# imulki/serenade

Measured on AMD Instinct MI355X. Metric: mel frames/sec converted (UNet ODE + vocoder), 80x1024, higher is better.
Workload: dtype f32

## Files before the change

### include/serenade_hip.h

```cpp
#ifndef SERENADE_HIP_H
#define SERENADE_HIP_H

#include <stdint.h>

#ifdef __cplusplus
extern "C" {
#endif

#define SRN_ABI_VERSION 4
#define SRN_MAX_TAPS 16

enum { SRN_ACT_NONE = 0, SRN_ACT_LEAKY = 1, SRN_ACT_SILU = 2, SRN_ACT_MISH = 3 };
enum { SRN_RES_NONE = 0, SRN_RES_ADD = 1, SRN_RES_AXPY = 2 };
enum {
  SRN_POST_NONE = 0,
  SRN_POST_DIV = 1,
  SRN_POST_TANH = 2,
  SRN_POST_RELU = 3,
  SRN_POST_LEAKY = 4,
  SRN_POST_GELU = 5
};
enum {
  SRN_PREC_FP32 = 0,
  SRN_PREC_BF16X3 = 1,
// ... 53 lines not shown
  void* ws; int64_t ws_bytes;
  const void* w_hi; const void* w_lo;
  float* gn_partials;
  float* out_tr; int64_t out_tr_bs; int32_t ld_out_tr; int32_t out_tr_col0;
} SrnConvParams;

int srn_abi_version(void);
const char* srn_last_error(void);

int srn_conv_gemm(const SrnConvParams* p, void* stream);
int64_t srn_conv_gemm_workspace_bytes(const SrnConvParams* p);
int srn_conv_gemm_route(const SrnConvParams* p, int32_t out[3]);
#define SRN_FORM_FIELDS 9
int srn_conv_gemm_forms(int32_t* rows, int capacity);

int srn_gn_mish_apply(const float* x, const float* gn_partials, const float* gamma, const float* beta,
                      const float* time_bias, int64_t time_bias_bs, const int32_t* lens, float* y, int B, int T,
                      int C, int groups, float eps, int valid_stats, void* stream);

int srn_resblock_tail(const float* c2, const float* gn_partials, const float* gamma, const float* beta,
                      const int32_t* lens, const float* r, const float* scale, const float* shift, int64_t ld_ss,
                      float* y, int B, int T, int C, int groups, float gn_eps, float ln_eps, int valid_stats,
                      void* stream);

int srn_resblock_tail_ln(const float* c2, const float* gn_partials, const float* gamma, const float* beta,
                         const int32_t* lens, const float* r, const float* scale, const float* shift, int64_t ld_ss,
                         float* y, int B, int T, int C, int groups, float gn_eps, float ln_eps, int valid_stats,
                         const float* ln2_gamma, const float* ln2_beta, float* y2, float ln2_eps, void* stream);

int srn_layernorm(const float* x, const float* gamma, const float* beta, float* y, int64_t rows, int C, float eps,
                  void* stream);

int srn_softmax_rows(float* s, const int32_t* lens, int Z, int n_head, int L, int ld, void* stream);

int srn_sinusoidal_emb(const float* t, float* out, int n, int dim, int ld, float scale, void* stream);

int srn_copy_channels(const float* src, int64_t src_bs, int ld_src, int sc0, float* dst, int64_t dst_bs, int ld_dst,
                      int dc0, int B, int T, int C, void* stream);

int srn_scatter_rows(const float* src, int64_t src_bs, int ld_src, float* dst, int64_t dst_bs, int ld_dst, int dc0,
                     const int32_t* row_off, const int32_t* n_rows, int B, int T, int C, void* stream);

int srn_transpose_ct(const float* src, float* dst, int B, int R, int Cc, int64_t src_bs, int ld_src, int64_t dst_bs,
                     int ld_dst, void* stream);
#define SRN_TR_LIST_MAX 40
typedef struct SrnTransposeList {
  int32_t n;
  int32_t pad_;
  const float* src[SRN_TR_LIST_MAX];
  float* dst[SRN_TR_LIST_MAX];
  int64_t src_bs[SRN_TR_LIST_MAX], dst_bs[SRN_TR_LIST_MAX];
  int32_t B[SRN_TR_LIST_MAX], R[SRN_TR_LIST_MAX], Cc[SRN_TR_LIST_MAX];
  int32_t ld_src[SRN_TR_LIST_MAX], ld_dst[SRN_TR_LIST_MAX];
  int32_t first_block[SRN_TR_LIST_MAX + 1];
} SrnTransposeList;
int srn_transpose_multi(const SrnTransposeList* list, void* stream);

int srn_renorm(const float* x, const float* trg_scale, const float* trg_mean, const float* voc_mean,
               const float* voc_scale, float* y, int64_t rows, int C, void* stream);

int srn_out_conv_tanh(const float* x, const float* w, const float* bias, float* y, int B, int T, int C, int k,
                      float slope, void* stream);
int srn_out_conv_tanh_ragged(const float* x, const float* w, const float* bias, float* y, const int32_t* lens, int B,
                             int T, int C, int k, float slope, void* stream);

typedef struct SrnResUnitParams {
// ... 256 lines not shown
```

### serenade_amd/_lib.py

```python
import collections
import ctypes
import os
from ctypes import POINTER, c_char_p, c_double, c_float, c_int, c_int32, c_int64, c_void_p

_HERE = os.path.dirname(os.path.abspath(__file__))
LIB_PATH = os.environ.get("SERENADE_AMD_LIB") or os.path.join(_HERE, "libserenade_hip.so")

SRN_MAX_TAPS = 16
ACT_NONE, ACT_LEAKY, ACT_SILU, ACT_MISH = 0, 1, 2, 3
RES_NONE, RES_ADD, RES_AXPY = 0, 1, 2
POST_NONE, POST_DIV, POST_TANH, POST_RELU, POST_LEAKY, POST_GELU = 0, 1, 2, 3, 4, 5
PREC_FP32, PREC_BF16X3, PREC_BF16X6 = 0, 1, 2
ROUTE_AUTO, ROUTE_TILED, ROUTE_HALO, ROUTE_GENERIC, ROUTE_STRIP, ROUTE_FAST_FP32 = 0, 1, 2, 3, 4, 5
FAMILY_GENERIC, FAMILY_F32, FAMILY_FAST, FAMILY_HALO, FAMILY_STRIP = 0, 1, 2, 3, 4
RESUNIT_ROUTE_SHARED = 1
TN_ROUTE_GENERAL = 1
RESUNIT_FORM_F32, RESUNIT_FORM_SHARED_F32, RESUNIT_FORM_BF16X3 = 0, 1, 2


class SrnConvParams(ctypes.Structure):
    _fields_ = [
        ("n_batch", c_int32), ("n_head", c_int32), ("T_in", c_int32), ("T_out", c_int32),
        ("C_in", c_int32), ("C_in0", c_int32), ("C_w", c_int32), ("N", c_int32), ("N_out", c_int32),
        ("n_taps", c_int32), ("tap_off", c_int32 * SRN_MAX_TAPS), ("in_stride", c_int32),
# ... 66 lines not shown
        ("route", c_int32),
    ]


class SrnExcitationParams(ctypes.Structure):
    _fields_ = [
        ("n_batch", c_int32), ("max_frames", c_int32), ("fs", c_int32), ("hop", c_int32),
        ("f0", c_void_p), ("df_f0", c_void_p), ("f_bs", c_int64), ("n_frames", c_void_p), ("phase_ws", c_void_p),
        ("noise", c_void_p), ("sine", c_void_p), ("sine_amp", c_float), ("noise_amp", c_float), ("n_df", c_int32),
        ("dfs", c_void_p * 4), ("df_upsample", c_int32 * 4), ("dense_factors", c_double * 4),
    ]


_P = c_void_p
_SIGS = {
    "srn_abi_version": (c_int, []),
    "srn_last_error": (c_char_p, []),
    "srn_conv_gemm": (c_int, [POINTER(SrnConvParams), _P]),
    "srn_conv_gemm_workspace_bytes": (c_int64, [POINTER(SrnConvParams)]),
    "srn_conv_gemm_route": (c_int, [POINTER(SrnConvParams), POINTER(c_int32)]),
    "srn_conv_gemm_forms": (c_int, [POINTER(c_int32), c_int]),
    "srn_hifigan_resunit": (c_int, [POINTER(SrnResUnitParams), _P]),
    "srn_hifigan_resunit_route": (c_int, [POINTER(SrnResUnitParams), POINTER(c_int32)]),
    "srn_hifigan_resunit_ragged": (c_int, [POINTER(SrnResUnitParams), _P, _P]),
    "srn_hifigan_resunit_ragged_route": (c_int, [POINTER(SrnResUnitParams), _P, POINTER(c_int32)]),
    "srn_gn_mish_apply": (c_int, [_P, _P, _P, _P, _P, c_int64, _P, _P, c_int, c_int, c_int, c_int, c_float, c_int, _P]),
    "srn_resblock_tail": (c_int, [_P, _P, _P, _P, _P, _P, _P, _P, c_int64, _P, c_int, c_int, c_int, c_int,
                                  c_float, c_float, c_int, _P]),
    "srn_resblock_tail_ln": (c_int, [_P, _P, _P, _P, _P, _P, _P, _P, c_int64, _P, c_int, c_int, c_int, c_int,
                                     c_float, c_float, c_int, _P, _P, _P, c_float, _P]),
    "srn_scatter_rows": (c_int, [_P, c_int64, c_int, _P, c_int64, c_int, c_int, _P, _P, c_int, c_int, c_int, _P]),
    "srn_layernorm": (c_int, [_P, _P, _P, _P, c_int64, c_int, c_float, _P]),
    "srn_softmax_rows": (c_int, [_P, _P, c_int, c_int, c_int, c_int, _P]),
    "srn_sinusoidal_emb": (c_int, [_P, _P, c_int, c_int, c_int, c_float, _P]),
    "srn_copy_channels": (c_int, [_P, c_int64, c_int, c_int, _P, c_int64, c_int, c_int, c_int, c_int, c_int, _P]),
    "srn_transpose_ct": (c_int, [_P, _P, c_int, c_int, c_int, c_int64, c_int, c_int64, c_int, _P]),
    "srn_transpose_multi": (c_int, [POINTER(SrnTransposeList), _P]),
    "srn_weight_norm_fwd": (c_int, [_P, _P, _P, _P, _P, c_int, c_int, c_int, _P]),
    "srn_weight_norm_bwd": (c_int, [_P, _P, _P, _P, _P, _P, c_int, c_int, c_int, _P]),
    "srn_renorm": (c_int, [_P, _P, _P, _P, _P, _P, c_int64, c_int, _P]),
    "srn_out_conv_tanh": (c_int, [_P, _P, _P, _P, c_int, c_int, c_int, c_int, c_float, _P]),
    "srn_out_conv_tanh_ragged": (c_int, [_P, _P, _P, _P, _P, c_int, c_int, c_int, c_int, c_float, _P]),
    "srn_pd_gather": (c_int, [_P, _P, _P, c_int, c_int, c_int, c_float, c_float, _P]),
    "srn_pd_gather_ragged": (c_int, [_P, _P, _P, _P, c_int, c_int, c_int, c_float, c_float, _P]),
    "srn_pad_signal": (c_int, [_P, _P, c_int, c_int, c_int, c_int, c_int, _P]),
    "srn_logmel": (c_int, [_P, _P, _P, c_int64, c_int, c_int, c_int, c_float, c_int, _P]),
    "srn_loudness": (c_int, [_P, _P, _P, _P, c_int, c_int, c_int, c_int, c_float, c_float, c_float, _P]),
    "srn_pad_ragged_zero": (c_int, [_P, c_int64, _P, _P, c_int, c_int, c_int, c_int, _P]),
    "srn_logmel_ragged": (c_int, [_P, _P, _P, _P, c_int, c_int, c_int, c_int, c_int, c_float, c_int, _P]),
    "srn_loudness_ragged": (c_int, [_P, _P, _P, _P, _P, c_int, c_int, c_int, c_int, c_float, c_float, c_float, _P]),
    "srn_gru_recur_last": (c_int, [_P, _P, _P, _P, c_int, c_int, c_int, _P]),
    "srn_style_token_attention_kv": (c_int, [_P] * 8 + [c_int] * 5 + [_P]),
    "srn_rowln_fwd": (c_int, [_P, _P, c_int64, _P, c_int64, _P, c_int, c_int, c_int, c_float, _P]),
    "srn_rowln_bwd": (c_int, [_P, _P, _P, c_int64, _P, _P, c_int, c_int, c_int, c_float, _P]),
    "srn_rowln_chunks": (c_int, [c_int]),
    "srn_gn_mish_bwd_partial": (c_int, [_P] * 8 + [c_int] * 4 + [_P]),
    "srn_gn_mish_bwd_apply": (c_int, [_P] * 9 + [c_int] * 4 + [_P]),
    "srn_gn_chunks": (c_int, [c_int]),
    "srn_gn_stats": (c_int, [_P, _P, _P, c_int, c_int, c_int, c_int, c_float, _P]),
    "srn_chunk_colsum": (c_int, [_P, _P, _P, _P, c_int, c_int, c_int, c_int, _P]),
    "srn_colsum": (c_int, [_P, _P, _P, c_int, c_int64, c_int, c_int, _P]),
    "srn_colsum_chunks": (c_int, [c_int64]),
    "srn_softmax_bwd": (c_int, [_P, _P, c_int64, c_int, c_int, c_float, _P]),
    "srn_geglu_fwd": (c_int, [_P, _P, c_int64, c_int, _P]),
    "srn_geglu_bwd": (c_int, [_P, _P, _P, c_int64, c_int, _P]),
    "srn_adamw": (c_int, [_P, _P, _P, _P, c_int64, c_float, c_float, c_float, c_float, c_float, c_int, c_float, _P]),
# ... 48 lines not shown
    "srn_note_decode": (c_int, [_P] * 4 + [c_int] * 3 + [c_float] * 2 + [c_int, c_double] + [_P] * 7),
    "srn_note_frames": (c_int, [_P] * 3 + [c_int] * 2 + [_P] + [c_double] * 3 + [_P] * 4 + [c_int] + [_P] * 3),
}

EXPORTS = tuple(_SIGS)

_lib = None


def lib():
    global _lib
    if _lib is None:
        if not os.path.exists(LIB_PATH):
            raise RuntimeError(
                f"{LIB_PATH} not found: build it with `python -m serenade_amd.build` "
                "(hipcc --offload-arch=gfx950). There is no CPU fallback.")
        h = ctypes.CDLL(LIB_PATH)
        for name, (res, args) in _SIGS.items():
            fn = getattr(h, name)
            fn.restype = res
            fn.argtypes = args
        if h.srn_abi_version() != 4:
            raise RuntimeError("libserenade_hip.so ABI version mismatch")
        _lib = h
    return _lib


def check(rc, what=""):
    if rc != 0:
        msg = lib().srn_last_error().decode("utf-8", "replace")
        raise RuntimeError(f"libserenade_hip {what} failed (rc={rc}): {msg}")


ConvForm = collections.namedtuple("ConvForm", "family tile precision nmajor kslices bm bn wn stages")


def conv_forms():
    k = len(ConvForm._fields)
    n = lib().srn_conv_gemm_forms(None, 0)
    rows = (c_int32 * (n * k))()
    assert lib().srn_conv_gemm_forms(rows, n) == n
    return [ConvForm(*rows[i * k:(i + 1) * k]) for i in range(n)]
```

### serenade_amd/csrc/norm_act.hip

```cpp
#include "common.h"
#include "conv_common.h"
#include "row_common.h"

namespace {

__device__ __forceinline__ void group_stats(const float* __restrict__ partials, int b, int T, int C, int groups,
                                            float eps, float* s_mean, float* s_rstd, int n_rows) {
  gn_group_stats(partials, b, T, C, groups, eps, n_rows,
                 [&](int g, float mean, float rstd) { s_mean[g] = mean, s_rstd[g] = rstd; });
  __syncthreads();
}

constexpr int GN_ROWS = 8;
constexpr int SMALL_GRID = 512;
constexpr int GN_PRE = 4;

__global__ __launch_bounds__(256) void gn_mish_apply_kernel(const float* __restrict__ x,
                                                            const float* __restrict__ partials,
                                                            const float* __restrict__ gamma,
                                                            const float* __restrict__ beta,
                                                            const float* __restrict__ time_bias,
                                                            const int32_t* __restrict__ lens, float* __restrict__ y,
                                                            int T, int C, int groups, float eps, int64_t tb_bs,
                                                            int valid_stats, int rows_per_wg) {
  __shared__ float s_mean[64], s_rstd[64];
  const int b = blockIdx.y;
  const int r0 = blockIdx.x * rows_per_wg;
  if (time_bias) time_bias += (int64_t)b * tb_bs;
  const int len = lens ? min(lens[b], T) : T;
  const int c4n = C / 4;
  const int cpg = C / groups;
  const int rows = min(rows_per_wg, T - r0);
  const int total = rows * c4n;
  const int64_t base = ((int64_t)b * T + r0) * C;
  float4 pre[GN_PRE];
#pragma unroll
  for (int k = 0; k < GN_PRE; ++k) {
    const int idx = threadIdx.x + 256 * k;
    pre[k] = make_float4(0.f, 0.f, 0.f, 0.f);
    if (idx < total) {
      const int r = idx / c4n;
      if (r0 + r < len) pre[k] = *reinterpret_cast<const float4*>(x + base + (int64_t)r * C + (idx - r * c4n) * 4);
    }
  }
  group_stats(partials, b, T, C, groups, eps, s_mean, s_rstd, valid_stats ? len : T);
  auto one = [&](const int idx, const float4 v) {
    const int r = idx / c4n;
    const int c = (idx - r * c4n) * 4;
    float4 o = make_float4(0.f, 0.f, 0.f, 0.f);
    if (r0 + r < len) {
      const float4 ga = *reinterpret_cast<const float4*>(gamma + c);
      const float4 be = *reinterpret_cast<const float4*>(beta + c);
      const int g = c / cpg;
      o = gn_mish4(v, s_mean[g], s_rstd[g], ga, be);
      if (time_bias) {
        const float4 tb = *reinterpret_cast<const float4*>(time_bias + c);
        o.x += tb.x;
        o.y += tb.y;
        o.z += tb.z;
        o.w += tb.w;
      }
    }
    *reinterpret_cast<float4*>(y + base + (int64_t)r * C + c) = o;
  };
#pragma unroll
  for (int k = 0; k < GN_PRE; ++k)
    if ((int)threadIdx.x + 256 * k < total) one(threadIdx.x + 256 * k, pre[k]);
  for (int idx = threadIdx.x + 256 * GN_PRE; idx < total; idx += 256) {
    const int r = idx / c4n;
    float4 v = make_float4(0.f, 0.f, 0.f, 0.f);
    if (r0 + r < len) v = *reinterpret_cast<const float4*>(x + base + (int64_t)r * C + (idx - r * c4n) * 4);
    one(idx, v);
  }
}

constexpr int TAIL_ROWS = 8;

__global__ __launch_bounds__(256) void resblock_tail_kernel(
    const float* __restrict__ c2, const float* __restrict__ partials, const float* __restrict__ gamma,
    const float* __restrict__ beta, const int32_t* __restrict__ lens, const float* __restrict__ rres,
    const float* __restrict__ scale, const float* __restrict__ shift, int64_t ld_ss, float* __restrict__ y, int T,
    int C, int groups, float gn_eps, float ln_eps, int valid_stats, const float* __restrict__ ln2_gamma,
    const float* __restrict__ ln2_beta, float* __restrict__ y2, float ln2_eps, int rows_per_wg) {
  __shared__ float s_mean[64], s_rstd[64];
  const int b = blockIdx.y;
  const int r0 = blockIdx.x * rows_per_wg;
  const int len = lens ? min(lens[b], T) : T;
  const int wave = threadIdx.x >> 6, lane = threadIdx.x & 63;
  const int c4n = C / 4;
  const int cpg = C / groups;
  const float inv_c = 1.0f / (float)C;
  const int r_end = min(r0 + rows_per_wg, T);
  float4 xin[MAXV], rin[MAXV];
  auto fetch = [&](const int r) {
    const int64_t row = ((int64_t)b * T + r) * C;
#pragma unroll
    for (int i = 0; i < MAXV; ++i) {
      const int c4 = lane + 64 * i;
      xin[i] = rin[i] = make_float4(0.f, 0.f, 0.f, 0.f);
      if (c4 < c4n) {
        rin[i] = *reinterpret_cast<const float4*>(rres + row + c4 * 4);
        if (r < len) xin[i] = *reinterpret_cast<const float4*>(c2 + row + c4 * 4);
      }
    }
  };
  if (r0 + wave < r_end) fetch(r0 + wave);
  group_stats(partials, b, T, C, groups, gn_eps, s_mean, s_rstd, valid_stats ? len : T);
  for (int r = r0 + wave; r < r_end; r += 4) {
    if (r != r0 + wave) fetch(r);
    const int64_t row = ((int64_t)b * T + r) * C;
    const bool valid = r < len;
    float4 v[MAXV];
#pragma unroll
    for (int i = 0; i < MAXV; ++i) {
      const int c4 = lane + 64 * i;
      v[i] = make_float4(0.f, 0.f, 0.f, 0.f);
      if (c4 < c4n) {
        const int c = c4 * 4;
        const float4 rr = rin[i];
        float4 o = make_float4(0.f, 0.f, 0.f, 0.f);
        if (valid) {
          const float4 ga = *reinterpret_cast<const float4*>(gamma + c);
          const float4 be = *reinterpret_cast<const float4*>(beta + c);
          const int g = c / cpg;
          o = gn_mish4(xin[i], s_mean[g], s_rstd[g], ga, be);
        }
        v[i] = make_float4(o.x + rr.x, o.y + rr.y, o.z + rr.z, o.w + rr.w);
      }
    }
    const float mean = row_sum(v, lane, c4n) * inv_c;
    const float stdv = sqrtf(row_sqdev(v, mean, lane, c4n) * inv_c + ln_eps);
    row_norm_affine_store<true>(v, mean, stdv, scale + (int64_t)b * ld_ss, shift + (int64_t)b * ld_ss, y + row, lane,
                                c4n);
    if (y2 != nullptr) row_layernorm_store(v, ln2_eps, ln2_gamma, ln2_beta, y2 + row, lane, c4n, inv_c);
  }
}

__global__ __launch_bounds__(256) void layernorm_kernel(const float* __restrict__ x, const float* __restrict__ gamma,
                                                        const float* __restrict__ beta, float* __restrict__ y,
                                                        int64_t rows, int C, float eps) {
  const int wave = threadIdx.x >> 6, lane = threadIdx.x & 63;
  const int c4n = C / 4;
  const float inv_c = 1.0f / (float)C;
  for (int64_t r = (int64_t)blockIdx.x * 4 + wave; r < rows; r += (int64_t)gridDim.x * 4) {
    float4 v[MAXV];
    row_load(x + r * C, v, lane, c4n);
    row_layernorm_store(v, eps, gamma, beta, y + r * C, lane, c4n, inv_c);
  }
}

template <int NV>
__global__ __launch_bounds__(256) void softmax_rows_kernel(float* __restrict__ s, const int32_t* __restrict__ lens,
                                                           int64_t n_rows, int n_head, int L, int ld) {
  const int wave = threadIdx.x >> 6, lane = threadIdx.x & 63;
  const int64_t r = (int64_t)blockIdx.x * 4 + wave;
  if (r >= n_rows) return;
  const int z = (int)(r / L);
  int len = L;
  if (lens) len = min(lens[z / n_head], L);
  float* row = s + r * ld;
  const int ld4 = ld / 4;
  float4 v[NV];
  float mx = -INFINITY;
#pragma unroll
  for (int i = 0; i < NV; ++i) {
    const int c4 = lane + 64 * i;
    v[i] = make_float4(-INFINITY, -INFINITY, -INFINITY, -INFINITY);
    if (c4 < ld4) {
      const float4 t = *reinterpret_cast<const float4*>(row + c4 * 4);
      const int c = c4 * 4;
      if (c + 0 < len) v[i].x = t.x;
      if (c + 1 < len) v[i].y = t.y;
      if (c + 2 < len) v[i].z = t.z;
      if (c + 3 < len) v[i].w = t.w;
      mx = fmaxf(mx, fmaxf(fmaxf(v[i].x, v[i].y), fmaxf(v[i].z, v[i].w)));
    }
  }
  mx = wave_max(mx);
  float sum = 0.f;
#pragma unroll
  for (int i = 0; i < NV; ++i) {
    if (lane + 64 * i < ld4) {
      v[i].x = expf(v[i].x - mx);
      v[i].y = expf(v[i].y - mx);
      v[i].z = expf(v[i].z - mx);
      v[i].w = expf(v[i].w - mx);
      sum += (v[i].x + v[i].y) + (v[i].z + v[i].w);
    }
  }
  sum = wave_sum(sum);
#pragma unroll
  for (int i = 0; i < NV; ++i) {
    const int c4 = lane + 64 * i;
    if (c4 < ld4) {
      float4 o;
      o.x = v[i].x / sum;
      o.y = v[i].y / sum;
      o.z = v[i].z / sum;
      o.w = v[i].w / sum;
      *reinterpret_cast<float4*>(row + c4 * 4) = o;
    }
  }
}

__global__ void sinusoidal_emb_kernel(const float* __restrict__ t, float* __restrict__ out, int n, int dim,
                                      int ld, float scale) {
  const int half = dim / 2;
  const int idx = blockIdx.x * blockDim.x + threadIdx.x;
  if (idx >= n * half) return;
  const int i = idx / half, k = idx - i * half;
  const float emb = logf(10000.0f) / (float)(half - 1);
  const float f = expf((float)k * -emb);
  const float arg = scale * t[i] * f;
  out[(int64_t)i * ld + k] = sinf(arg);
  out[(int64_t)i * ld + half + k] = cosf(arg);
}

__global__ void copy_channels_kernel(const float* __restrict__ src, int64_t src_bs, int ld_src, int sc0,
                                     float* __restrict__ dst, int64_t dst_bs, int ld_dst, int dc0, int T, int C) {
  const int b = blockIdx.y;
  const int64_t total = (int64_t)T * C;
  for (int64_t idx = (int64_t)blockIdx.x * blockDim.x + threadIdx.x; idx < total;
       idx += (int64_t)gridDim.x * blockDim.x) {
    const int t = (int)(idx / C), c = (int)(idx - (int64_t)t * C);
    dst[(int64_t)b * dst_bs + (int64_t)t * ld_dst + dc0 + c] = src[(int64_t)b * src_bs + (int64_t)t * ld_src + sc0 + c];
  }
}

__global__ void scatter_rows_kernel(const float* __restrict__ src, int64_t src_bs, int ld_src,
                                    float* __restrict__ dst, int64_t dst_bs, int ld_dst, int dc0,
                                    const int32_t* __restrict__ row_off, const int32_t* __restrict__ n_rows, int T,
                                    int C) {
  const int b = blockIdx.y;
  const int off = row_off ? row_off[b] : 0;
  const int64_t total = (int64_t)min(n_rows ? n_rows[b] : T, T) * C;
// ... 135 lines not shown
  const int t = blockIdx.x * 256 + threadIdx.x;
  if (t >= T) return;
  int L = T;
  if constexpr (RAGGED) {
    L = max(min(srn_first(lens...)[b], T), 0);
    if (t >= L) {
      y[(int64_t)b * T + t] = 0.f;
      return;
    }
  }
  const float* xb = x + (int64_t)b * T * C;
  float acc = bias[0];
  for (int j = 0; j < K; ++j) {
    const int ti = t + j - (K - 1) / 2;
    if (ti < 0 || ti >= L) continue;
    for (int c = 0; c < C; ++c) {
      float v = xb[(int64_t)ti * C + c];
      v = v > 0.f ? v : v * slope;
      acc = fmaf(v, w[j * C + c], acc);
    }
  }
  y[(int64_t)b * T + t] = tanhf(acc);
}

}

extern "C" int srn_gn_mish_apply(const float* x, const float* gn_partials, const float* gamma, const float* beta,
                                 const float* time_bias, int64_t time_bias_bs, const int32_t* lens, float* y, int B,
                                 int T, int C, int groups, float eps, int valid_stats, void* stream) {
  SRN_CHECK_ARG(x && gn_partials && gamma && beta && y, "gn_mish_apply: null pointer");
  SRN_CHECK_ARG(!valid_stats || lens, "gn_mish_apply: valid_stats needs lens");
  SRN_CHECK_ARG(B > 0 && T > 0 && C > 0 && groups > 0 && groups <= 64 && C % groups == 0 && (C / groups) % 32 == 0,
                "gn_mish_apply: need (C / groups) %% 32 == 0 (C=%d groups=%d)", C, groups);
  const int rows_per_wg = (int64_t)B * ((T + GN_ROWS - 1) / GN_ROWS) < SMALL_GRID ? GN_ROWS / 2 : GN_ROWS;
  dim3 grid((T + rows_per_wg - 1) / rows_per_wg, B);
  hipLaunchKernelGGL(gn_mish_apply_kernel, grid, dim3(256), 0, (hipStream_t)stream, x, gn_partials, gamma, beta,
                     time_bias, lens, y, T, C, groups, eps, time_bias_bs, valid_stats, rows_per_wg);
  SRN_CHECK_LAUNCH();
  return 0;
}

static int resblock_tail_launch(const char* name, const float* c2, const float* gn_partials, const float* gamma,
                                const float* beta, const int32_t* lens, const float* r, const float* scale,
                                const float* shift, int64_t ld_ss, float* y, int B, int T, int C, int groups, float gn_eps,
                                float ln_eps, int valid_stats, const float* ln2_gamma, const float* ln2_beta, float* y2,
                                float ln2_eps, void* stream) {
  SRN_CHECK_ARG(c2 && gn_partials && gamma && beta && r && scale && shift && y, "%s: null pointer", name);
  SRN_CHECK_ARG(!valid_stats || lens, "%s: valid_stats needs lens", name);
  SRN_CHECK_ARG(B > 0 && T > 0 && C > 0 && C % 4 == 0 && C <= 256 * MAXV, "%s: C=%d unsupported", name, C);
  SRN_CHECK_ARG(groups > 0 && groups <= 64 && C % groups == 0 && (C / groups) % 32 == 0,
                "%s: need (C / groups) %% 32 == 0", name);
  const int rows_per_wg = (int64_t)B * ((T + TAIL_ROWS - 1) / TAIL_ROWS) < SMALL_GRID ? TAIL_ROWS / 2 : TAIL_ROWS;
  dim3 grid((T + rows_per_wg - 1) / rows_per_wg, B);
  hipLaunchKernelGGL(resblock_tail_kernel, grid, dim3(256), 0, (hipStream_t)stream, c2, gn_partials, gamma, beta,
                     lens, r, scale, shift, ld_ss, y, T, C, groups, gn_eps, ln_eps, valid_stats, ln2_gamma, ln2_beta,
                     y2, ln2_eps, rows_per_wg);
  SRN_CHECK_LAUNCH();
  return 0;
}

extern "C" int srn_resblock_tail(const float* c2, const float* gn_partials, const float* gamma, const float* beta,
                                 const int32_t* lens, const float* r, const float* scale, const float* shift,
                                 int64_t ld_ss, float* y, int B, int T, int C, int groups, float gn_eps,
                                 float ln_eps, int valid_stats, void* stream) {
  return resblock_tail_launch("resblock_tail", c2, gn_partials, gamma, beta, lens, r, scale, shift, ld_ss, y, B, T, C,
                              groups, gn_eps, ln_eps, valid_stats, nullptr, nullptr, nullptr, 0.f, stream);
}

extern "C" int srn_resblock_tail_ln(const float* c2, const float* gn_partials, const float* gamma, const float* beta,
                                    const int32_t* lens, const float* r, const float* scale, const float* shift,
                                    int64_t ld_ss, float* y, int B, int T, int C, int groups, float gn_eps,
                                    float ln_eps, int valid_stats, const float* ln2_gamma, const float* ln2_beta,
                                    float* y2, float ln2_eps, void* stream) {
  SRN_CHECK_ARG(ln2_gamma && ln2_beta && y2, "resblock_tail_ln: null pointer");
  return resblock_tail_launch("resblock_tail_ln", c2, gn_partials, gamma, beta, lens, r, scale, shift, ld_ss, y, B, T,
                              C, groups, gn_eps, ln_eps, valid_stats, ln2_gamma, ln2_beta, y2, ln2_eps, stream);
}

extern "C" int srn_layernorm(const float* x, const float* gamma, const float* beta, float* y, int64_t rows, int C,
                             float eps, void* stream) {
  SRN_CHECK_ARG(x && gamma && beta && y, "layernorm: null pointer");
  SRN_CHECK_ARG(rows > 0 && C > 0 && C % 4 == 0 && C <= 256 * MAXV, "layernorm: C=%d unsupported", C);
  int64_t blocks = (rows + 3) / 4;
  if (blocks > 65536) blocks = 65536;
  hipLaunchKernelGGL(layernorm_kernel, dim3((unsigned)blocks), dim3(256), 0, (hipStream_t)stream, x, gamma, beta, y,
                     rows, C, eps);
  SRN_CHECK_LAUNCH();
  return 0;
}

extern "C" int srn_softmax_rows(float* s, const int32_t* lens, int Z, int n_head, int L, int ld, void* stream) {
  SRN_CHECK_ARG(s != nullptr && Z > 0 && n_head > 0 && L > 0 && ld >= L && ld % 4 == 0, "softmax_rows: bad args");
  const int64_t rows = (int64_t)Z * L;
  const unsigned blocks = (unsigned)((rows + 3) / 4);
  const int nv = (ld / 4 + 63) / 64;
  hipStream_t st = (hipStream_t)stream;
  if (nv <= 2) hipLaunchKernelGGL(softmax_rows_kernel<2>, dim3(blocks), dim3(256), 0, st, s, lens, rows, n_head, L, ld);
  else if (nv <= 4) hipLaunchKernelGGL(softmax_rows_kernel<4>, dim3(blocks), dim3(256), 0, st, s, lens, rows, n_head, L, ld);
  else if (nv <= 8) hipLaunchKernelGGL(softmax_rows_kernel<8>, dim3(blocks), dim3(256), 0, st, s, lens, rows, n_head, L, ld);
  else if (nv <= 12) hipLaunchKernelGGL(softmax_rows_kernel<12>, dim3(blocks), dim3(256), 0, st, s, lens, rows, n_head, L, ld);
  else if (nv <= 20) hipLaunchKernelGGL(softmax_rows_kernel<20>, dim3(blocks), dim3(256), 0, st, s, lens, rows, n_head, L, ld);
  else if (nv <= 36) hipLaunchKernelGGL(softmax_rows_kernel<36>, dim3(blocks), dim3(256), 0, st, s, lens, rows, n_head, L, ld);
  else {
    srn_set_error("softmax_rows: ld=%d too long (max 9216)", ld);
    return -1;
  }
  SRN_CHECK_LAUNCH();
  return 0;
}

extern "C" int srn_sinusoidal_emb(const float* t, float* out, int n, int dim, int ld, float scale, void* stream) {
  SRN_CHECK_ARG(t && out && n > 0 && dim > 2 && dim % 2 == 0 && ld >= dim, "sinusoidal_emb: bad args");
  const int total = n * (dim / 2);
  hipLaunchKernelGGL(sinusoidal_emb_kernel, dim3((total + 255) / 256), dim3(256), 0, (hipStream_t)stream, t, out, n,
                     dim, ld, scale);
  SRN_CHECK_LAUNCH();
  return 0;
}

extern "C" int srn_copy_channels(const float* src, int64_t src_bs, int ld_src, int sc0, float* dst, int64_t dst_bs,
                                 int ld_dst, int dc0, int B, int T, int C, void* stream) {
  SRN_CHECK_ARG(src && dst && B > 0 && T > 0 && C > 0, "copy_channels: bad args");
  int64_t blocks = ((int64_t)T * C + 255) / 256;
  if (blocks > 4096) blocks = 4096;
  hipLaunchKernelGGL(copy_channels_kernel, dim3((unsigned)blocks, B), dim3(256), 0, (hipStream_t)stream, src, src_bs,
                     ld_src, sc0, dst, dst_bs, ld_dst, dc0, T, C);
  SRN_CHECK_LAUNCH();
  return 0;
}

extern "C" int srn_scatter_rows(const float* src, int64_t src_bs, int ld_src, float* dst, int64_t dst_bs, int ld_dst,
                                int dc0, const int32_t* row_off, const int32_t* n_rows, int B, int T, int C,
                                void* stream) {
  SRN_CHECK_ARG(src && dst && B > 0 && T > 0 && C > 0, "scatter_rows: bad args");
  int64_t blocks = ((int64_t)T * C + 255) / 256;
  if (blocks > 1024) blocks = 1024;
  hipLaunchKernelGGL(scatter_rows_kernel, dim3((unsigned)blocks, B), dim3(256), 0, (hipStream_t)stream, src, src_bs,
                     ld_src, dst, dst_bs, ld_dst, dc0, row_off, n_rows, T, C);
  SRN_CHECK_LAUNCH();
  return 0;
// ... 132 lines not shown
```

### serenade_amd/csrc/row_common.h

```cpp
#pragma once
#include "common.h"

template <class F>
__device__ __forceinline__ float4 map4(float4 v, F f) {
  return make_float4(f(v.x), f(v.y), f(v.z), f(v.w));
}
__device__ __forceinline__ float hsum4(float4 v) { return (v.x + v.y) + (v.z + v.w); }
__device__ __forceinline__ float4 mul4(float4 a, float4 b) { return make_float4(a.x * b.x, a.y * b.y, a.z * b.z, a.w * b.w); }
__device__ __forceinline__ float sqdev4(float4 v, float mean) {
  const float dx = v.x - mean, dy = v.y - mean, dz = v.z - mean, dw = v.w - mean;
  return (dx * dx + dy * dy) + (dz * dz + dw * dw);
}
template <bool DIV = false>
__device__ __forceinline__ float4 xhat4(float4 v, float mean, float s) {
  return map4(v, [=](float t) { return DIV ? (t - mean) / s : (t - mean) * s; });
}
__device__ __forceinline__ float4 affine4(float4 h, float4 g, float4 b) {
  return make_float4(h.x * g.x + b.x, h.y * g.y + b.y, h.z * g.z + b.z, h.w * g.w + b.w);
}
template <bool DIV = false>
__device__ __forceinline__ float4 norm_affine4(float4 v, float mean, float s, float4 g, float4 b) {
  return affine4(xhat4<DIV>(v, mean, s), g, b);
}

// ... 11 lines not shown
  float sum = 0.f;
#pragma unroll
  for (int i = 0; i < MAXV; ++i)
    if (lane + 64 * i < c4n) sum += hsum4(v[i]);
  return wave_sum(sum);
}
__device__ __forceinline__ float row_sqdev(const float4 (&v)[MAXV], float mean, int lane, int c4n) {
  float sq = 0.f;
#pragma unroll
  for (int i = 0; i < MAXV; ++i)
    if (lane + 64 * i < c4n) sq += sqdev4(v[i], mean);
  return wave_sum(sq);
}
template <bool DIV = false>
__device__ __forceinline__ void row_norm_affine_store(float4 (&v)[MAXV], float mean, float s, const float* __restrict__ g,
                                                      const float* __restrict__ b, float* __restrict__ y, int lane,
                                                      int c4n) {
#pragma unroll
  for (int i = 0; i < MAXV; ++i) {
    const int c = (lane + 64 * i) * 4;
    if (c < c4n * 4) {
      v[i] = norm_affine4<DIV>(v[i], mean, s, *reinterpret_cast<const float4*>(g + c),
                               *reinterpret_cast<const float4*>(b + c));
      *reinterpret_cast<float4*>(y + c) = v[i];
    }
  }
}
__device__ __forceinline__ void row_layernorm_store(float4 (&v)[MAXV], float eps, const float* __restrict__ g,
                                                    const float* __restrict__ b, float* __restrict__ y, int lane,
                                                    int c4n, float inv_c) {
  const float mean = row_sum(v, lane, c4n) * inv_c;
  const float rstd = 1.0f / sqrtf(row_sqdev(v, mean, lane, c4n) * inv_c + eps);
  row_norm_affine_store(v, mean, rstd, g, b, y, lane, c4n);
}

template <class Store>
__device__ __forceinline__ void gn_group_stats(const float* __restrict__ partials, int b, int T, int C, int groups,
                                               float eps, int n_rows, Store store) {
  const int gn_mt = (T + 31) / 32;
  const int gn_nt = C / 32;
  const int nt_per_g = (C / groups) / 32;
  const int wave = threadIdx.x >> 6, lane = threadIdx.x & 63;
  const float* base = partials + (int64_t)b * gn_mt * gn_nt * 2;
  const int per_g = gn_mt * nt_per_g;
  for (int g = wave; g < groups; g += 4) {
    double s1 = 0.0, s2 = 0.0;
    for (int e = lane; e < per_g; e += 64) {
      const int mt = e / nt_per_g;
      const int nt = g * nt_per_g + (e - mt * nt_per_g);
      const float2 v = *reinterpret_cast<const float2*>(base + ((int64_t)mt * gn_nt + nt) * 2);
      s1 += (double)v.x;
      s2 += (double)v.y;
    }
    s1 = wave_sum_d(s1);
    s2 = wave_sum_d(s2);
    if (lane == 0) {
      const double cnt = (double)max(n_rows, 1) * (double)(C / groups);
      const double mean = s1 / cnt;
      double var = s2 / cnt - mean * mean;
      if (var < 0.0) var = 0.0;
      store(g, (float)mean, (float)(1.0 / sqrt(var + (double)eps)));
    }
  }
}
__device__ __forceinline__ float4 gn_mish4(float4 x, float m, float rs, float4 ga, float4 be) {
  return map4(norm_affine4(x, m, rs, ga, be), [](float t) { return srn_mish(t); });
// ... 85 lines not shown
```

Baseline: 62380.

## Software-pipeline row-pass kernels with prefetch ring and register-cached params

```diff
diff --git a/include/serenade_hip.h b/include/serenade_hip.h
--- a/include/serenade_hip.h
+++ b/include/serenade_hip.h
@@ -109,6 +109,13 @@
                   void* stream);
 
 int srn_softmax_rows(float* s, const int32_t* lens, int Z, int n_head, int L, int ld, void* stream);
+
+#define SRN_ROWPASS_GN_MISH_APPLY 0
+#define SRN_ROWPASS_RESBLOCK_TAIL 1
+#define SRN_ROWPASS_LAYERNORM 2
+#define SRN_ROWPASS_SOFTMAX_ROWS 3
+#define SRN_ROWPASS_FIELDS 6
+int srn_row_pass_geometry(int op, int B, int64_t rows, int C, int32_t* out);
 
 int srn_sinusoidal_emb(const float* t, float* out, int n, int dim, int ld, float scale, void* stream);
 
diff --git a/serenade_amd/_lib.py b/serenade_amd/_lib.py
--- a/serenade_amd/_lib.py
+++ b/serenade_amd/_lib.py
@@ -122,6 +122,7 @@
     "srn_scatter_rows": (c_int, [_P, c_int64, c_int, _P, c_int64, c_int, c_int, _P, _P, c_int, c_int, c_int, _P]),
     "srn_layernorm": (c_int, [_P, _P, _P, _P, c_int64, c_int, c_float, _P]),
     "srn_softmax_rows": (c_int, [_P, _P, c_int, c_int, c_int, c_int, _P]),
+    "srn_row_pass_geometry": (c_int, [c_int, c_int, c_int64, c_int, POINTER(c_int32)]),
     "srn_sinusoidal_emb": (c_int, [_P, _P, c_int, c_int, c_int, c_float, _P]),
     "srn_copy_channels": (c_int, [_P, c_int64, c_int, c_int, _P, c_int64, c_int, c_int, c_int, c_int, c_int, _P]),
     "srn_transpose_ct": (c_int, [_P, _P, c_int, c_int, c_int, c_int64, c_int, c_int64, c_int, _P]),
@@ -236,6 +237,16 @@
         raise RuntimeError(f"libserenade_hip {what} failed (rc={rc}): {msg}")
 
 
+ROWPASS_GN_MISH_APPLY, ROWPASS_RESBLOCK_TAIL, ROWPASS_LAYERNORM, ROWPASS_SOFTMAX_ROWS = 0, 1, 2, 3
+RowPass = collections.namedtuple("RowPass", "rows_per_wg grid_x grid_y in_flight grid_cap softmax_nv")
+
+
+def row_pass_geometry(op, B, rows, C):
+    out = (c_int32 * len(RowPass._fields))()
+    check(lib().srn_row_pass_geometry(op, B, rows, C, out), "srn_row_pass_geometry")
+    return RowPass(*out)
+
+
 ConvForm = collections.namedtuple("ConvForm", "family tile precision nmajor kslices bm bn wn stages")
 
 
diff --git a/serenade_amd/csrc/norm_act.hip b/serenade_amd/csrc/norm_act.hip
--- a/serenade_amd/csrc/norm_act.hip
+++ b/serenade_amd/csrc/norm_act.hip
@@ -1,6 +1,8 @@
 #include "common.h"
 #include "conv_common.h"
 #include "row_common.h"
+
+#include <algorithm>
 
 namespace {
 
@@ -15,7 +17,89 @@
 constexpr int SMALL_GRID = 512;
 constexpr int GN_PRE = 4;
 
+constexpr int SMALL_ROWS = 4;
+constexpr int STREAM_ROWS = 32;
+constexpr int STREAM_GRID = 512;
+
+int64_t ceil_div(int64_t a, int64_t b) { return (a + b - 1) / b; }
+
+int stream_rows_per_wg(int B, int T) {
+  return (int)std::min<int64_t>(STREAM_ROWS, std::max<int64_t>(SMALL_ROWS, 4 * ceil_div((int64_t)B * T, 4 * STREAM_GRID)));
+}
+
+template <int NV>
+__device__ __forceinline__ void param_load(const float* __restrict__ p, float4 (&v)[MAXV], int lane, int c4n) {
+#pragma unroll
+  for (int i = 0; i < MAXV; ++i) {
+    v[i] = make_float4(0.f, 0.f, 0.f, 0.f);
+    if (i < NV && p != nullptr && lane + 64 * i < c4n) v[i] = *reinterpret_cast<const float4*>(p + (lane + 64 * i) * 4);
+  }
+}
+
+struct GnRow {
+  float4 x[MAXV];
+};
+
+template <int NV>
 __global__ __launch_bounds__(256) void gn_mish_apply_kernel(const float* __restrict__ x,
+                                                            const float* __restrict__ partials,
+                                                            const float* __restrict__ gamma,
+                                                            const float* __restrict__ beta,
+                                                            const float* __restrict__ time_bias,
+                                                            const int32_t* __restrict__ lens, float* __restrict__ y,
+                                                            int T, int C, int groups, float eps, int64_t tb_bs,
+                                                            int valid_stats, int rows_per_wg) {
+  __shared__ float s_mean[64], s_rstd[64];
+  const int b = blockIdx.y;
+  const int r0 = blockIdx.x * rows_per_wg;
+  const int len = lens ? min(lens[b], T) : T;
+  const int wave = srn_wave(), lane = threadIdx.x & 63;
+  const int c4n = min(C / 4, 64 * NV);
+  const int r_end = min(r0 + rows_per_wg, T);
+  const int64_t item = (int64_t)b * T * C;
+  auto load = [&](const int64_t r, GnRow& q) {
+#pragma unroll
+    for (int i = 0; i < NV; ++i) {
+      q.x[i] = make_float4(0.f, 0.f, 0.f, 0.f);
+      if (lane + 64 * i < c4n && r < len) q.x[i] = *reinterpret_cast<const float4*>(x + item + r * C + (lane + 64 * i) * 4);
+    }
+  };
+  GnRow ring[ROWS_AHEAD];
+  rows_prime(ring, r0 + wave, r_end, 4, load);
+  float4 ga[MAXV], be[MAXV], tb[MAXV];
+  param_load<NV>(gamma, ga, lane, c4n);
+  param_load<NV>(beta, be, lane, c4n);
+  param_load<NV>(time_bias ? time_bias + (int64_t)b * tb_bs : nullptr, tb, lane, c4n);
+  group_stats(partials, b, T, C, groups, eps, s_mean, s_rstd, valid_stats ? len : T);
+  float gm[NV], gr[NV];
+  const int cpg = C / groups;
+#pragma unroll
+  for (int i = 0; i < NV; ++i) {
+    const int g = min((lane + 64 * i) * 4 / cpg, groups - 1);
+    gm[i] = s_mean[g], gr[i] = s_rstd[g];
+  }
+  rows_walk(ring, r0 + wave, r_end, 4, load, [&](const int64_t r, const GnRow& q) {
+    const bool valid = r < len;
+#pragma unroll
+    for (int i = 0; i < NV; ++i) {
+      if (lane + 64 * i < c4n) {
+        float4 o = make_float4(0.f, 0.f, 0.f, 0.f);
+        if (valid) {
+          o = gn_mish4(q.x[i], gm[i], gr[i], ga[i], be[i]);
+          if (time_bias) {
+            o.x += tb[i].x;
+            o.y += tb[i].y;
+            o.z += tb[i].z;
+            o.w += tb[i].w;
+          }
+        }
+        *reinterpret_cast<float4*>(y + item + r * C + (lane + 64 * i) * 4) = o;
+      }
+    }
+  });
+}
+
+__global__ __launch_bounds__(256) void gn_mish_apply_flat_kernel(const float* __restrict__ x,
                                                             const float* __restrict__ partials,
                                                             const float* __restrict__ gamma,
                                                             const float* __restrict__ beta,
@@ -74,8 +158,11 @@
   }
 }
 
-constexpr int TAIL_ROWS = 8;
-
+struct TailRow {
+  float4 x[MAXV], r[MAXV];
+};
+
+template <int NV>
 __global__ __launch_bounds__(256) void resblock_tail_kernel(
     const float* __restrict__ c2, const float* __restrict__ partials, const float* __restrict__ gamma,
     const float* __restrict__ beta, const int32_t* __restrict__ lens, const float* __restrict__ rres,
@@ -86,80 +173,101 @@
   const int b = blockIdx.y;
   const int r0 = blockIdx.x * rows_per_wg;
   const int len = lens ? min(lens[b], T) : T;
-  const int wave = threadIdx.x >> 6, lane = threadIdx.x & 63;
-  const int c4n = C / 4;
-  const int cpg = C / groups;
+  const int wave = srn_wave(), lane = threadIdx.x & 63;
+  const int c4n = min(C / 4, 64 * NV);
   const float inv_c = 1.0f / (float)C;
   const int r_end = min(r0 + rows_per_wg, T);
-  float4 xin[MAXV], rin[MAXV];
-  auto fetch = [&](const int r) {
-    const int64_t row = ((int64_t)b * T + r) * C;
-#pragma unroll
-    for (int i = 0; i < MAXV; ++i) {
+  const int64_t item = (int64_t)b * T * C;
+  auto load = [&](const int64_t r, TailRow& q) {
+#pragma unroll
+    for (int i = 0; i < NV; ++i) {
       const int c4 = lane + 64 * i;
-      xin[i] = rin[i] = make_float4(0.f, 0.f, 0.f, 0.f);
+      q.x[i] = q.r[i] = make_float4(0.f, 0.f, 0.f, 0.f);
       if (c4 < c4n) {
-        rin[i] = *reinterpret_cast<const float4*>(rres + row + c4 * 4);
-        if (r < len) xin[i] = *reinterpret_cast<const float4*>(c2 + row + c4 * 4);
+        q.r[i] = *reinterpret_cast<const float4*>(rres + item + r * C + c4 * 4);
+        if (r < len) q.x[i] = *reinterpret_cast<const float4*>(c2 + item + r * C + c4 * 4);
       }
     }
   };
-  if (r0 + wave < r_end) fetch(r0 + wave);
+  TailRow ring[ROWS_AHEAD];
+  rows_prime(ring, r0 + wave, r_end, 4, load);
+  float4 ga[MAXV], be[MAXV], sc[MAXV], sh[MAXV], g2[MAXV], b2[MAXV];
+  param_load<NV>(gamma, ga, lane, c4n);
+  param_load<NV>(beta, be, lane, c4n);
+  param_load<NV>(scale + (int64_t)b * ld_ss, sc, lane, c4n);
+  param_load<NV>(shift + (int64_t)b * ld_ss, sh, lane, c4n);
+  param_load<NV>(ln2_gamma, g2, lane, c4n);
+  param_load<NV>(ln2_beta, b2, lane, c4n);
   group_stats(partials, b, T, C, groups, gn_eps, s_mean, s_rstd, valid_stats ? len : T);
-  for (int r = r0 + wave; r < r_end; r += 4) {
-    if (r != r0 + wave) fetch(r);
-    const int64_t row = ((int64_t)b * T + r) * C;
+  float gm[NV], gr[NV];
+  const int cpg = C / groups;
+#pragma unroll
+  for (int i = 0; i < NV; ++i) {
+    const int g = min((lane + 64 * i) * 4 / cpg, groups - 1);
+    gm[i] = s_mean[g], gr[i] = s_rstd[g];
+  }
+  rows_walk(ring, r0 + wave, r_end, 4, load, [&](const int64_t r, const TailRow& q) {
+    const int64_t row = item + r * C;
     const bool valid = r < len;
     float4 v[MAXV];
 #pragma unroll
     for (int i = 0; i < MAXV; ++i) {
-      const int c4 = lane + 64 * i;
       v[i] = make_float4(0.f, 0.f, 0.f, 0.f);
-      if (c4 < c4n) {
-        const int c = c4 * 4;
-        const float4 rr = rin[i];
+      if (i < NV && lane + 64 * i < c4n) {
+        const float4 rr = q.r[i];
         float4 o = make_float4(0.f, 0.f, 0.f, 0.f);
-        if (valid) {
-          const float4 ga = *reinterpret_cast<const float4*>(gamma + c);
-          const float4 be = *reinterpret_cast<const float4*>(beta + c);
-          const int g = c / cpg;
-          o = gn_mish4(xin[i], s_mean[g], s_rstd[g], ga, be);
-        }
+        if (valid) o = gn_mish4(q.x[i], gm[i], gr[i], ga[i], be[i]);
         v[i] = make_float4(o.x + rr.x, o.y + rr.y, o.z + rr.z, o.w + rr.w);
       }
     }
     const float mean = row_sum(v, lane, c4n) * inv_c;
     const float stdv = sqrtf(row_sqdev(v, mean, lane, c4n) * inv_c + ln_eps);
-    row_norm_affine_store<true>(v, mean, stdv, scale + (int64_t)b * ld_ss, shift + (int64_t)b * ld_ss, y + row, lane,
-                                c4n);
-    if (y2 != nullptr) row_layernorm_store(v, ln2_eps, ln2_gamma, ln2_beta, y2 + row, lane, c4n, inv_c);
-  }
-}
-
+    row_norm_affine_store<true>(v, mean, stdv, sc, sh, y + row, lane, c4n);
+    if (y2 != nullptr) row_layernorm_store(v, ln2_eps, g2, b2, y2 + row, lane, c4n, inv_c);
+  });
+}
+
+constexpr int LN_GRID_CAP = 2048;
+
+struct LnRow {
+  float4 v[MAXV];
+};
+
+template <int NV>
 __global__ __launch_bounds__(256) void layernorm_kernel(const float* __restrict__ x, const float* __restrict__ gamma,
                                                         const float* __restrict__ beta, float* __restrict__ y,
                                                         int64_t rows, int C, float eps) {
-  const int wave = threadIdx.x >> 6, lane = threadIdx.x & 63;
-  const int c4n = C / 4;
+  const int wave = srn_wave(), lane = threadIdx.x & 63;
+  const int c4n = min(C / 4, 64 * NV);
   const float inv_c = 1.0f / (float)C;
-  for (int64_t r = (int64_t)blockIdx.x * 4 + wave; r < rows; r += (int64_t)gridDim.x * 4) {
-    float4 v[MAXV];
-    row_load(x + r * C, v, lane, c4n);
-    row_layernorm_store(v, eps, gamma, beta, y + r * C, lane, c4n, inv_c);
-  }
+  const int64_t first = (int64_t)blockIdx.x * 4 + wave, step = (int64_t)gridDim.x * 4;
+  auto load = [&](const int64_t r, LnRow& q) {
+#pragma unroll
+    for (int i = 0; i < MAXV; ++i) {
+      q.v[i] = make_float4(0.f, 0.f, 0.f, 0.f);
+      if (i < NV && lane + 64 * i < c4n) q.v[i] = *reinterpret_cast<const float4*>(x + r * C + (lane + 64 * i) * 4);
+    }
+  };
+  LnRow ring[ROWS_AHEAD];
+  rows_prime(ring, first, rows, step, load);
+  float4 ga[MAXV], be[MAXV];
+  param_load<NV>(gamma, ga, lane, c4n);
+  param_load<NV>(beta, be, lane, c4n);
+  rows_walk(ring, first, rows, step, load,
+            [&](const int64_t r, LnRow& q) { row_layernorm_store(q.v, eps, ga, be, y + r * C, lane, c4n, inv_c); });
 }
 
 template <int NV>
-__global__ __launch_bounds__(256) void softmax_rows_kernel(float* __restrict__ s, const int32_t* __restrict__ lens,
-                                                           int64_t n_rows, int n_head, int L, int ld) {
-  const int wave = threadIdx.x >> 6, lane = threadIdx.x & 63;
-  const int64_t r = (int64_t)blockIdx.x * 4 + wave;
-  if (r >= n_rows) return;
-  const int z = (int)(r / L);
-  int len = L;
-  if (lens) len = min(lens[z / n_head], L);
-  float* row = s + r * ld;
-  const int ld4 = ld / 4;
+__device__ __forceinline__ void softmax_row_load(const float* __restrict__ row, float4 (&t)[NV], int lane, int ld4) {
+#pragma unroll
+  for (int i = 0; i < NV; ++i) {
+    t[i] = make_float4(-INFINITY, -INFINITY, -INFINITY, -INFINITY);
+    if (lane + 64 * i < ld4) t[i] = *reinterpret_cast<const float4*>(row + (lane + 64 * i) * 4);
+  }
+}
+template <int NV>
+__device__ __forceinline__ void softmax_row_store(float* __restrict__ row, const float4 (&t)[NV], int len, int lane,
+                                                  int ld4) {
   float4 v[NV];
   float mx = -INFINITY;
 #pragma unroll
@@ -167,12 +275,11 @@
     const int c4 = lane + 64 * i;
     v[i] = make_float4(-INFINITY, -INFINITY, -INFINITY, -INFINITY);
     if (c4 < ld4) {
-      const float4 t = *reinterpret_cast<const float4*>(row + c4 * 4);
       const int c = c4 * 4;
-      if (c + 0 < len) v[i].x = t.x;
-      if (c + 1 < len) v[i].y = t.y;
-      if (c + 2 < len) v[i].z = t.z;
-      if (c + 3 < len) v[i].w = t.w;
+      if (c + 0 < len) v[i].x = t[i].x;
+      if (c + 1 < len) v[i].y = t[i].y;
+      if (c + 2 < len) v[i].z = t[i].z;
+      if (c + 3 < len) v[i].w = t[i].w;
       mx = fmaxf(mx, fmaxf(fmaxf(v[i].x, v[i].y), fmaxf(v[i].z, v[i].w)));
     }
   }
@@ -201,6 +308,20 @@
       *reinterpret_cast<float4*>(row + c4 * 4) = o;
     }
   }
+}
+
+template <int NV>
+__global__ __launch_bounds__(256) void softmax_rows_kernel(float* __restrict__ s, const int32_t* __restrict__ lens,
+                                                           int64_t n_rows, int n_head, int L, int ld) {
+  const int wave = srn_wave(), lane = threadIdx.x & 63;
+  const int64_t r = (int64_t)blockIdx.x * 4 + wave;
+  if (r >= n_rows) return;
+  const int z = (int)(r / L);
+  int len = L;
+  if (lens) len = min(lens[z / n_head], L);
+  float4 t[NV];
+  softmax_row_load<NV>(s + r * ld, t, lane, ld / 4);
+  softmax_row_store<NV>(s + r * ld, t, len, lane, ld / 4);
 }
 
 __global__ void sinusoidal_emb_kernel(const float* __restrict__ t, float* __restrict__ out, int n, int dim,
@@ -402,10 +523,19 @@
   SRN_CHECK_ARG(!valid_stats || lens, "gn_mish_apply: valid_stats needs lens");
   SRN_CHECK_ARG(B > 0 && T > 0 && C > 0 && groups > 0 && groups <= 64 && C % groups == 0 && (C / groups) % 32 == 0,
                 "gn_mish_apply: need (C / groups) %% 32 == 0 (C=%d groups=%d)", C, groups);
-  const int rows_per_wg = (int64_t)B * ((T + GN_ROWS - 1) / GN_ROWS) < SMALL_GRID ? GN_ROWS / 2 : GN_ROWS;
-  dim3 grid((T + rows_per_wg - 1) / rows_per_wg, B);
-  hipLaunchKernelGGL(gn_mish_apply_kernel, grid, dim3(256), 0, (hipStream_t)stream, x, gn_partials, gamma, beta,
-                     time_bias, lens, y, T, C, groups, eps, time_bias_bs, valid_stats, rows_per_wg);
+  int32_t geo[SRN_ROWPASS_FIELDS];
+  if (srn_row_pass_geometry(SRN_ROWPASS_GN_MISH_APPLY, B, T, C, geo) != 0) return -1;
+  const int rows_per_wg = geo[0];
+  dim3 grid(geo[1], geo[2]);
+  hipStream_t st = (hipStream_t)stream;
+#define SRN_GN_LAUNCH(kernel)                                                                                        \
+  hipLaunchKernelGGL(kernel, grid, dim3(256), 0, st, x, gn_partials, gamma, beta, time_bias, lens, y, T, C, groups, \
+                     eps, time_bias_bs, valid_stats, rows_per_wg)
+  if (C <= 256) SRN_GN_LAUNCH(gn_mish_apply_kernel<1>);
+  else if (C <= 512) SRN_GN_LAUNCH(gn_mish_apply_kernel<2>);
+  else if (C <= 256 * MAXV) SRN_GN_LAUNCH(gn_mish_apply_kernel<4>);
+  else SRN_GN_LAUNCH(gn_mish_apply_flat_kernel);
+#undef SRN_GN_LAUNCH
   SRN_CHECK_LAUNCH();
   return 0;
 }
@@ -420,11 +550,18 @@
   SRN_CHECK_ARG(B > 0 && T > 0 && C > 0 && C % 4 == 0 && C <= 256 * MAXV, "%s: C=%d unsupported", name, C);
   SRN_CHECK_ARG(groups > 0 && groups <= 64 && C % groups == 0 && (C / groups) % 32 == 0,
                 "%s: need (C / groups) %% 32 == 0", name);
-  const int rows_per_wg = (int64_t)B * ((T + TAIL_ROWS - 1) / TAIL_ROWS) < SMALL_GRID ? TAIL_ROWS / 2 : TAIL_ROWS;
-  dim3 grid((T + rows_per_wg - 1) / rows_per_wg, B);
-  hipLaunchKernelGGL(resblock_tail_kernel, grid, dim3(256), 0, (hipStream_t)stream, c2, gn_partials, gamma, beta,
-                     lens, r, scale, shift, ld_ss, y, T, C, groups, gn_eps, ln_eps, valid_stats, ln2_gamma, ln2_beta,
-                     y2, ln2_eps, rows_per_wg);
+  int32_t geo[SRN_ROWPASS_FIELDS];
+  if (srn_row_pass_geometry(SRN_ROWPASS_RESBLOCK_TAIL, B, T, C, geo) != 0) return -1;
+  const int rows_per_wg = geo[0];
+  dim3 grid(geo[1], geo[2]);
+  hipStream_t st = (hipStream_t)stream;
+#define SRN_TAIL_LAUNCH(NV)                                                                                         \
+  hipLaunchKernelGGL(resblock_tail_kernel<NV>, grid, dim3(256), 0, st, c2, gn_partials, gamma, beta, lens, r, scale, \
+                     shift, ld_ss, y, T, C, groups, gn_eps, ln_eps, valid_stats, ln2_gamma, ln2_beta, y2, ln2_eps,    \
+                     rows_per_wg)
+  if (C <= 512) SRN_TAIL_LAUNCH(2);
+  else SRN_TAIL_LAUNCH(4);
+#undef SRN_TAIL_LAUNCH
   SRN_CHECK_LAUNCH();
   return 0;
 }
@@ -451,10 +588,11 @@
                              float eps, void* stream) {
   SRN_CHECK_ARG(x && gamma && beta && y, "layernorm: null pointer");
   SRN_CHECK_ARG(rows > 0 && C > 0 && C % 4 == 0 && C <= 256 * MAXV, "layernorm: C=%d unsupported", C);
-  int64_t blocks = (rows + 3) / 4;
-  if (blocks > 65536) blocks = 65536;
-  hipLaunchKernelGGL(layernorm_kernel, dim3((unsigned)blocks), dim3(256), 0, (hipStream_t)stream, x, gamma, beta, y,
-                     rows, C, eps);
+  int32_t geo[SRN_ROWPASS_FIELDS];
+  if (srn_row_pass_geometry(SRN_ROWPASS_LAYERNORM, 1, rows, C, geo) != 0) return -1;
+  hipStream_t st = (hipStream_t)stream;
+  if (C <= 512) hipLaunchKernelGGL(layernorm_kernel<2>, dim3(geo[1]), dim3(256), 0, st, x, gamma, beta, y, rows, C, eps);
+  else hipLaunchKernelGGL(layernorm_kernel<4>, dim3(geo[1]), dim3(256), 0, st, x, gamma, beta, y, rows, C, eps);
   SRN_CHECK_LAUNCH();
   return 0;
 }
@@ -462,20 +600,59 @@
 extern "C" int srn_softmax_rows(float* s, const int32_t* lens, int Z, int n_head, int L, int ld, void* stream) {
   SRN_CHECK_ARG(s != nullptr && Z > 0 && n_head > 0 && L > 0 && ld >= L && ld % 4 == 0, "softmax_rows: bad args");
   const int64_t rows = (int64_t)Z * L;
-  const unsigned blocks = (unsigned)((rows + 3) / 4);
-  const int nv = (ld / 4 + 63) / 64;
+  int32_t geo[SRN_ROWPASS_FIELDS];
+  if (srn_row_pass_geometry(SRN_ROWPASS_SOFTMAX_ROWS, 1, rows, ld, geo) != 0) return -1;
+  const dim3 blocks(geo[1]);
   hipStream_t st = (hipStream_t)stream;
-  if (nv <= 2) hipLaunchKernelGGL(softmax_rows_kernel<2>, dim3(blocks), dim3(256), 0, st, s, lens, rows, n_head, L, ld);
-  else if (nv <= 4) hipLaunchKernelGGL(softmax_rows_kernel<4>, dim3(blocks), dim3(256), 0, st, s, lens, rows, n_head, L, ld);
-  else if (nv <= 8) hipLaunchKernelGGL(softmax_rows_kernel<8>, dim3(blocks), dim3(256), 0, st, s, lens, rows, n_head, L, ld);
-  else if (nv <= 12) hipLaunchKernelGGL(softmax_rows_kernel<12>, dim3(blocks), dim3(256), 0, st, s, lens, rows, n_head, L, ld);
-  else if (nv <= 20) hipLaunchKernelGGL(softmax_rows_kernel<20>, dim3(blocks), dim3(256), 0, st, s, lens, rows, n_head, L, ld);
-  else if (nv <= 36) hipLaunchKernelGGL(softmax_rows_kernel<36>, dim3(blocks), dim3(256), 0, st, s, lens, rows, n_head, L, ld);
-  else {
-    srn_set_error("softmax_rows: ld=%d too long (max 9216)", ld);
-    return -1;
-  }
-  SRN_CHECK_LAUNCH();
+#define SRN_SM_LAUNCH(kernel) hipLaunchKernelGGL(kernel, blocks, dim3(256), 0, st, s, lens, rows, n_head, L, ld)
+  switch (geo[5]) {
+    case 2: SRN_SM_LAUNCH(softmax_rows_kernel<2>); break;
+    case 4: SRN_SM_LAUNCH(softmax_rows_kernel<4>); break;
+    case 8: SRN_SM_LAUNCH(softmax_rows_kernel<8>); break;
+    case 12: SRN_SM_LAUNCH(softmax_rows_kernel<12>); break;
+    case 20: SRN_SM_LAUNCH(softmax_rows_kernel<20>); break;
+    default: SRN_SM_LAUNCH(softmax_rows_kernel<36>); break;
+  }
+#undef SRN_SM_LAUNCH
+  SRN_CHECK_LAUNCH();
+  return 0;
+}
+
+extern "C" int srn_row_pass_geometry(int op, int B, int64_t rows, int C, int32_t* out) {
+  SRN_CHECK_ARG(out != nullptr && B > 0 && rows > 0 && C > 0, "row_pass_geometry: bad args");
+  int64_t r_wg = 4, gx = 1, gy = 1, in_flight = ROWS_AHEAD + 1, cap = 0, nv = 0;
+  switch (op) {
+    case SRN_ROWPASS_GN_MISH_APPLY:
+    case SRN_ROWPASS_RESBLOCK_TAIL:
+      SRN_CHECK_ARG(rows < (1ll << 31), "row_pass_geometry: T too large");
+      if (op == SRN_ROWPASS_GN_MISH_APPLY && C > 256 * MAXV) {
+        r_wg = (int64_t)B * ceil_div(rows, GN_ROWS) < SMALL_GRID ? GN_ROWS / 2 : GN_ROWS;
+        in_flight = 1;
+      } else {
+        r_wg = stream_rows_per_wg(B, (int)rows);
+      }
+      gx = ceil_div(rows, r_wg), gy = B;
+      break;
+    case SRN_ROWPASS_LAYERNORM:
+      cap = LN_GRID_CAP;
+      gx = std::min<int64_t>(ceil_div(rows, 4), cap);
+      break;
+    case SRN_ROWPASS_SOFTMAX_ROWS:
+      nv = (C / 4 + 63) / 64;
+      nv = nv <= 2 ? 2 : nv <= 4 ? 4 : nv <= 8 ? 8 : nv <= 12 ? 12 : nv <= 20 ? 20 : nv <= 36 ? 36 : -1;
+      if (nv < 0) {
+        srn_set_error("softmax_rows: ld=%d too long (max 9216)", C);
+        return -1;
+      }
+      gx = ceil_div(rows, 4), in_flight = 1;
+      SRN_CHECK_ARG(gx < (1ll << 31), "softmax_rows: too many rows");
+      break;
+    default:
+      srn_set_error("row_pass_geometry: unknown op %d", op);
+      return -1;
+  }
+  out[0] = (int32_t)r_wg, out[1] = (int32_t)gx, out[2] = (int32_t)gy, out[3] = (int32_t)in_flight;
+  out[4] = (int32_t)cap, out[5] = (int32_t)nv;
   return 0;
 }
 
diff --git a/serenade_amd/csrc/row_common.h b/serenade_amd/csrc/row_common.h
--- a/serenade_amd/csrc/row_common.h
+++ b/serenade_amd/csrc/row_common.h
@@ -67,6 +67,54 @@
   const float mean = row_sum(v, lane, c4n) * inv_c;
   const float rstd = 1.0f / sqrtf(row_sqdev(v, mean, lane, c4n) * inv_c + eps);
   row_norm_affine_store(v, mean, rstd, g, b, y, lane, c4n);
+}
+
+template <bool DIV = false>
+__device__ __forceinline__ void row_norm_affine_store(float4 (&v)[MAXV], float mean, float s, const float4 (&g)[MAXV],
+                                                      const float4 (&b)[MAXV], float* __restrict__ y, int lane,
+                                                      int c4n) {
+#pragma unroll
+  for (int i = 0; i < MAXV; ++i) {
+    const int c = (lane + 64 * i) * 4;
+    if (c < c4n * 4) {
+      v[i] = norm_affine4<DIV>(v[i], mean, s, g[i], b[i]);
+      *reinterpret_cast<float4*>(y + c) = v[i];
+    }
+  }
+}
+__device__ __forceinline__ void row_layernorm_store(float4 (&v)[MAXV], float eps, const float4 (&g)[MAXV],
+                                                    const float4 (&b)[MAXV], float* __restrict__ y, int lane, int c4n,
+                                                    float inv_c) {
+  const float mean = row_sum(v, lane, c4n) * inv_c;
+  const float rstd = 1.0f / sqrtf(row_sqdev(v, mean, lane, c4n) * inv_c + eps);
+  row_norm_affine_store(v, mean, rstd, g, b, y, lane, c4n);
+}
+
+constexpr int ROWS_AHEAD = 1;
+
+__device__ __forceinline__ int srn_wave() { return __builtin_amdgcn_readfirstlane((int)(threadIdx.x >> 6)); }
+
+template <class Row, class Load>
+__device__ __forceinline__ void rows_prime(Row (&ring)[ROWS_AHEAD], int64_t first, int64_t end, int64_t step,
+                                           Load load) {
+#pragma unroll
+  for (int k = 0; k < ROWS_AHEAD; ++k)
+    if (first + k * step < end) load(first + k * step, ring[k]);
+}
+template <class Row, class Load, class Body>
+__device__ __forceinline__ void rows_walk(Row (&ring)[ROWS_AHEAD], int64_t first, int64_t end, int64_t step, Load load,
+                                          Body body) {
+  for (int64_t r = first; r < end; r += ROWS_AHEAD * step) {
+#pragma unroll
+    for (int k = 0; k < ROWS_AHEAD; ++k) {
+      const int64_t rk = r + k * step;
+      if (rk < end) {
+        Row cur = ring[k];
+        if (rk + ROWS_AHEAD * step < end) load(rk + ROWS_AHEAD * step, ring[k]);
+        body(rk, cur);
+      }
+    }
+  }
 }
 
 template <class Store>
```

Result: no change. 62660 (median of 6 runs) (+0.4%).
